# a1q123456/image_stitching

Measured on AMD Instinct MI355X. Metric: 4K frames stitched/sec, higher is better.
Workload: dtype u8

## Files before the change

image_stitching_amd/csrc/orb.hip:

```cpp
#include "common.h"
#include "dev_math.h"
#include <algorithm>
#include <chrono>
#include <cmath>

#define ORB_MAX_LEVELS 16
#define ORB_BORDER 32

namespace {

struct LevelDesc {
    int w, h;
    int pp;
    int sp;
    size_t pad_off;
    size_t map_off;
    float scale;
    int nfeat;
    int n2;
    int tiles_x, tiles_y, tile_off;
    int cap1, cand_off;
    int cap2, fin_off;
    int tab_off;
};
// ... 312 lines not shown
#pragma unroll
        for (int k = 0; k < FT_WR + 1; k++) {
            if ((ball[k] >> lane) & 1ull) {
                const int r = k < FT_WR ? r0 + k : r0 + (lane >> 1), c = k < FT_WR ? lane : FT_COLS + (lane & 1);
                queue[base + __popcll(ball[k] & below)] = (unsigned short)(r * (FT_COLS + 2) + c);
            }
            base += __popcll(ball[k]);
        }
    }
    __syncthreads();
    for (int q = t; q < qcount; q += 256) {
        const int i = queue[q], r = i / (FT_COLS + 2), c = i - r * (FT_COLS + 2);
        const int fsv = fast_score_full(g + (r + 3) * FG_PITCH + (c + FG_COL0), FG_PITCH, L.fast_t);
        sc[r * SP + c] = (uint8_t)fsv;
#ifdef MIS_ORB_STATS
        if (fsv) atomicAdd(&g_orb_stats[3], 1ull);
#endif
    }
    __syncthreads();
    lh[t] = 0;
    {
        const int nq = qcount;
        for (int q0 = 0; q0 < nq; q0 += 256) {
            const int q = q0 + t;
            bool keep = false;
            int x = 0, y = 0, v = 0;
            if (q < nq) {
                const int i = queue[q], r = i / (FT_COLS + 2), c = i - r * (FT_COLS + 2);
                const uint8_t* s_ = sc + r * SP + c;
                v = s_[0];
                x = x0 - 1 + c; y = y0 - 1 + r;
                keep = v && r >= 1 && r <= FT_ROWS && c >= 1 && c <= FT_COLS && x >= L.edge && x < d.w - L.edge && y >= L.edge && y < d.h - L.edge &&
                       v > s_[-1] && v > s_[1] && v > s_[-SP - 1] && v > s_[-SP] && v > s_[-SP + 1] && v > s_[SP - 1] && v > s_[SP] && v > s_[SP + 1];
            }
            const unsigned long long m = __ballot(keep);
            int base = 0;
            if ((t & 63) == 0 && m) base = atomicAdd(&lcount, __popcll(m));
            base = __shfl(base, 0);
            if (keep) {
                const int j = base + __popcll(m & ((1ull << (t & 63)) - 1ull));
                lxy[j] = (uint32_t)x | ((uint32_t)y << 16); lsc[j] = (uint8_t)v;
            }
        }
    }
    __syncthreads();
    const int n = lcount;
    const int tile = d.tile_off + blockIdx.y * d.tiles_x + blockIdx.x;
    if (t == 0) tile_cnt[tile] = n;
    if (n == 0) return;
    for (int j = t; j < n; j += 256) {
        atomicAdd(&lh[lsc[j]], 1);
        surv_xy[(size_t)tile * FT_SLOTS + j] = lxy[j]; surv_sc[(size_t)tile * FT_SLOTS + j] = lsc[j];
    }
    __syncthreads();
    if (lh[t]) atomicAdd(&hist[((lz * HIST_COPIES) + ((blockIdx.x + blockIdx.y) & (HIST_COPIES - 1))) * 256 + t], lh[t]);
}

__global__ __launch_bounds__(256) void fast_cut_kernel(Levels L, const int* hist, int* thr, int* flags, size_t ws) {
    __shared__ int suf[256];
    __shared__ int s_thr;
    const int l = blockIdx.x, t = threadIdx.x;
    WS_OFF(hist, blockIdx.y, ws); WS_OFF(thr, blockIdx.y, ws); WS_OFF(flags, blockIdx.y, ws);
    const LevelDesc& d = L.d[l];
    int hsum = 0;
    for (int c = 0; c < HIST_COPIES; c++) hsum += hist[(l * HIST_COPIES + c) * 256 + t];
    suf[t] = t ? hsum : 0;
    __syncthreads();
    for (int o = 1; o < 256; o <<= 1) {
        int add = t + o < 256 ? suf[t + o] : 0;
        __syncthreads();
        suf[t] += add;
        __syncthreads();
    }
    if (t == 0) s_thr = d.n2 == 0 ? 256 : 1;
    __syncthreads();
    if (d.n2 > 0 && suf[1] > d.n2 && t >= 1 && suf[t] >= d.n2 && (t == 255 || suf[t + 1] < d.n2)) s_thr = t;
    __syncthreads();
    if (t == 0) {
        thr[l] = s_thr;
        if (s_thr < 256 && suf[s_thr] > d.cap1) atomicOr(&flags[0], 1);
    }
}

constexpr int CT_TILES = 16;
__global__ __launch_bounds__(256) void compact_kernel(Levels L, const int* tile_cnt, const uint32_t* surv_xy, const uint8_t* surv_sc, const int* thr,
                                                      int* cnt1, uint32_t* cand_xy, float* cand_resp, size_t ws) {
    __shared__ int s_cnt[CT_TILES], s_off[CT_TILES];
    __shared__ int s_base;
    const int l = blockIdx.y, t = threadIdx.x, lane = t & 63, wave = t >> 6;
    WS_OFF(tile_cnt, blockIdx.z, ws); WS_OFF(surv_xy, blockIdx.z, ws); WS_OFF(surv_sc, blockIdx.z, ws); WS_OFF(thr, blockIdx.z, ws);
    WS_OFF(cnt1, blockIdx.z, ws); WS_OFF(cand_xy, blockIdx.z, ws); WS_OFF(cand_resp, blockIdx.z, ws);
    const LevelDesc& d = L.d[l];
    const int ntiles = d.tiles_x * d.tiles_y, first = blockIdx.x * CT_TILES;
    if (first >= ntiles) return;
    const int th = thr[l];
    for (int k = 0; k < CT_TILES / 4; k++) {
        const int slot = wave * (CT_TILES / 4) + k, til = first + slot;
        int cnt = 0;
        if (til < ntiles) {
            const int tile = d.tile_off + til, n = tile_cnt[tile];
            for (int j0 = 0; j0 < n; j0 += 64) {
                const int j = j0 + lane;
                const int v = j < n ? surv_sc[(size_t)tile * FT_SLOTS + j] : 0;
                cnt += __popcll(__ballot(v >= th && v > 0));
            }
        }
        if (lane == 0) s_cnt[slot] = cnt;
    }
    __syncthreads();
    if (t == 0) {
        int tot = 0;
        for (int k = 0; k < CT_TILES; k++) { s_off[k] = tot; tot += s_cnt[k]; }
        s_base = tot ? atomicAdd(&cnt1[l], tot) : 0;
    }
    __syncthreads();
    for (int k = 0; k < CT_TILES / 4; k++) {
        const int slot = wave * (CT_TILES / 4) + k, til = first + slot;
        if (til >= ntiles || s_cnt[slot] == 0) continue;
        const int tile = d.tile_off + til, n = tile_cnt[tile];
        int run = s_base + s_off[slot];
        for (int j0 = 0; j0 < n; j0 += 64) {
            const int j = j0 + lane;
            const int v = j < n ? surv_sc[(size_t)tile * FT_SLOTS + j] : 0;
            const bool keep = v >= th && v > 0;
            const unsigned long long m = __ballot(keep);
            if (keep) {
                const int i = run + __popcll(m & ((1ull << lane) - 1ull));
                if (i < d.cap1) { cand_xy[d.cand_off + i] = surv_xy[(size_t)tile * FT_SLOTS + j]; cand_resp[d.cand_off + i] = (float)v; }
            }
            run += __popcll(m);
        }
    }
}

__global__ void nms_raster_kernel(LevelDesc d, const int* tile_cnt, const uint32_t* surv_xy, const uint8_t* surv_sc, uint8_t* nms) {
    const int ntiles = d.tiles_x * d.tiles_y;
    for (int tl = blockIdx.x; tl < ntiles; tl += gridDim.x) {
        const int tile = d.tile_off + tl, n = tile_cnt[tile];
        for (int j = threadIdx.x; j < n; j += blockDim.x) {
            uint32_t xy = surv_xy[(size_t)tile * FT_SLOTS + j];
            nms[d.map_off + (size_t)(xy >> 16) * d.sp + (xy & 0xffff)] = surv_sc[(size_t)tile * FT_SLOTS + j];
        }
    }
}

__global__ __launch_bounds__(256) void harris_kernel(Levels L, const uint8_t* pad, const int* cnt1, const uint32_t* cand_xy, float* cand_resp, size_t ws) {
    const LevelDesc& d = L.d[blockIdx.y];
    WS_OFF(pad, blockIdx.z, ws); WS_OFF(cnt1, blockIdx.z, ws); WS_OFF(cand_xy, blockIdx.z, ws); WS_OFF(cand_resp, blockIdx.z, ws);
    int i = blockIdx.x * 256 + threadIdx.x;
    int n = min(cnt1[blockIdx.y], d.cap1);
    if (i >= n) return;
    uint32_t xy = cand_xy[d.cand_off + i];
    int x = xy & 0xffff, y = xy >> 16;
    const int pp = d.pp;
    const uint8_t* q0 = pad + d.pad_off + (size_t)(y + ORB_BORDER - 4) * pp + (x + ORB_BORDER - 4);
    const unsigned sh = (unsigned)((uintptr_t)q0 & 3u);
    const uint8_t* a0 = q0 - sh;
    int px[9][9];
#pragma unroll
    for (int r = 0; r < 9; r++) {
        const unsigned* row = reinterpret_cast<const unsigned*>(a0 + (size_t)r * pp);
        const unsigned d0 = row[0], d1 = row[1], d2 = row[2];
        const unsigned w0 = __builtin_amdgcn_alignbyte(d1, d0, sh), w1 = __builtin_amdgcn_alignbyte(d2, d1, sh), w2 = __builtin_amdgcn_alignbyte(0u, d2, sh);
#pragma unroll
        for (int k = 0; k < 4; k++) { px[r][k] = (int)((w0 >> (8 * k)) & 255u); px[r][4 + k] = (int)((w1 >> (8 * k)) & 255u); }
        px[r][8] = (int)(w2 & 255u);
    }
    int a = 0, b = 0, c = 0;
#pragma unroll
    for (int by = 0; by < 7; by++)
#pragma unroll
        for (int bx = 0; bx < 7; bx++) {
            const int Ix = (px[by + 1][bx + 2] - px[by + 1][bx]) * 2 + (px[by][bx + 2] - px[by][bx]) + (px[by + 2][bx + 2] - px[by + 2][bx]);
            const int Iy = (px[by + 2][bx + 1] - px[by][bx + 1]) * 2 + (px[by + 2][bx] - px[by][bx]) + (px[by + 2][bx + 2] - px[by][bx + 2]);
            a += Ix * Ix; b += Iy * Iy; c += Ix * Iy;
        }
    const float scale = 1.f / ((1 << 2) * 7 * 255.f);
    const float scale_sq_sq = scale * scale * scale * scale;
    float fa = (float)a, fb = (float)b, fc = (float)c;
    float s1 = fa * fb, s2 = fc * fc;
    float s3 = 0.04f * (fa + fb);
    s3 = s3 * (fa + fb);
    cand_resp[d.cand_off + i] = ((s1 - s2) - s3) * scale_sq_sq;
}

__device__ __forceinline__ uint32_t fkey(float f) {
    uint32_t u = __float_as_uint(f);
    return (u & 0x80000000u) ? ~u : (u | 0x80000000u);
}

__global__ __launch_bounds__(1024) void select_rank_kernel(Levels L, const int* cnt1, const uint32_t* cand_xy, const float* cand_resp,
                                                            int* cnt2, uint32_t* fin_xy, float* fin_resp, int* flags, int use_harris, size_t ws) {
    WS_OFF(cnt1, blockIdx.y, ws); WS_OFF(cand_xy, blockIdx.y, ws); WS_OFF(cand_resp, blockIdx.y, ws); WS_OFF(cnt2, blockIdx.y, ws);
    WS_OFF(fin_xy, blockIdx.y, ws); WS_OFF(fin_resp, blockIdx.y, ws); WS_OFF(flags, blockIdx.y, ws);
    __shared__ int hist[256];
    __shared__ uint32_t s_prefix, s_mask;
    __shared__ int s_k, s_m;
    __shared__ uint32_t kkey[4096], kxy[4096];
    const int l = blockIdx.x, t = threadIdx.x;
    const LevelDesc& d = L.d[l];
    const int n = min(cnt1[l], d.cap1);
    const uint32_t* xy = cand_xy + d.cand_off;
    const float* rs = cand_resp + d.cand_off;
    const int N = d.nfeat;
    if (N == 0) { if (t == 0) cnt2[l] = 0; return; }
    if (n <= 4096) {
        int P = 1;
        while (P < n) P <<= 1;
        for (int i = t; i < P; i += 1024) {
            if (i < n) { kkey[i] = fkey(rs[i]); kxy[i] = xy[i]; }
            else { kkey[i] = 0; kxy[i] = 0xffffffffu; }
        }
        __syncthreads();
        for (int k = 2; k <= P; k <<= 1)
            for (int j = k >> 1; j > 0; j >>= 1) {
                for (int i = t; i < P; i += 1024) {
                    const int ixj = i ^ j;
                    if (ixj > i) {
                        const uint32_t ka = kkey[i], kb = kkey[ixj], pa = kxy[i], pb = kxy[ixj];
                        const bool a_first = ka > kb || (ka == kb && pa < pb);
                        const bool descending_block = (i & k) == 0;
                        if (a_first != descending_block) { kkey[i] = kb; kkey[ixj] = ka; kxy[i] = pb; kxy[ixj] = pa; }
                    }
                }
                __syncthreads();
            }
        const uint32_t cutk = (use_harris && n > N) ? kkey[N - 1] : 0u;
        if (t == 0) s_m = 0;
        __syncthreads();
        for (int i = t; i < n; i += 1024)
            if (kkey[i] >= cutk && (i == n - 1 || kkey[i + 1] < cutk)) s_m = i + 1;
        __syncthreads();
        const int m = s_m;
        if (m > d.cap2) { if (t == 0) { atomicOr(&flags[0], 2); cnt2[l] = 0; } return; }
        for (int i = t; i < m; i += 1024) {
            fin_xy[d.fin_off + i] = kxy[i];
            const uint32_t ki = kkey[i], uu = (ki & 0x80000000u) ? (ki & 0x7fffffffu) : ~ki;
            fin_resp[d.fin_off + i] = __uint_as_float(uu);
        }
        if (t == 0) cnt2[l] = m;
        return;
    }
    uint32_t cut = 0;
    if (use_harris && n > N) {
        if (t == 0) { s_prefix = 0; s_mask = 0; s_k = N; }
        __syncthreads();
        for (int shift = 24; shift >= 0; shift -= 8) {
            if (t < 256) hist[t] = 0;
            __syncthreads();
            uint32_t prefix = s_prefix, mask = s_mask;
            for (int i = t; i < n; i += 1024) {
                uint32_t k = fkey(rs[i]);
                if ((k & mask) == prefix) atomicAdd(&hist[(k >> shift) & 255], 1);
            }
            __syncthreads();
            if (t == 0) {
                int k = s_k, b = 255;
                for (; b > 0; b--) { if (hist[b] >= k) break; k -= hist[b]; }
                s_k = k; s_prefix = prefix | ((uint32_t)b << shift); s_mask = mask | (0xffu << shift);
            }
            __syncthreads();
        }
        cut = s_prefix;
    }
    if (t == 0) s_m = 0;
    __syncthreads();
    for (int i = t; i < n; i += 1024) {
        uint32_t k = fkey(rs[i]);
        if (k >= cut) {
            int j = atomicAdd(&s_m, 1);
            if (j < 4096) { kkey[j] = k; kxy[j] = xy[i]; }
        }
    }
    __syncthreads();
    int m = s_m;
    if (m > d.cap2 || m > 4096) { if (t == 0) { atomicOr(&flags[0], 2); cnt2[l] = 0; } return; }
    for (int i = t; i < m; i += 1024) {
        uint32_t ki = kkey[i], pi = kxy[i];
        uint32_t yi = (pi >> 16), xi = pi & 0xffff;
        uint32_t oi = (yi << 16) | xi;
        int r = 0;
        for (int j = 0; j < m; j++) {
            uint32_t kj = kkey[j], pj = kxy[j];
            uint32_t oj = ((pj >> 16) << 16) | (pj & 0xffff);
            r += (kj > ki) || (kj == ki && oj < oi);
        }
        fin_xy[d.fin_off + r] = pi;
        uint32_t u = (ki & 0x80000000u) ? (ki & 0x7fffffffu) : ~ki;
        fin_resp[d.fin_off + r] = __uint_as_float(u);
    }
    if (t == 0) cnt2[l] = m;
}

__global__ __launch_bounds__(256) void assemble_kernel(Levels L, const int* cnt2, const uint32_t* fin_xy, const float* fin_resp, OrbIO io, int cap_out, size_t ws) {
    const int fr = blockIdx.y;
    WS_OFF(cnt2, fr, ws); WS_OFF(fin_xy, fr, ws); WS_OFF(fin_resp, fr, ws);
    MisKeyPoint* kps = io.kps[fr];
    int* n_out = io.n_dev[fr];
    const int j = blockIdx.x * 4 + (threadIdx.x >> 6), lane = threadIdx.x & 63;
    int base = 0, l = 0, total = 0;
    {
        int c[ORB_MAX_LEVELS];
#pragma unroll
        for (int k = 0; k < ORB_MAX_LEVELS; k++) c[k] = k < L.n ? cnt2[min(k, L.n - 1)] : 0;
#pragma unroll
        for (int k = 0; k < ORB_MAX_LEVELS; k++) {
            if (j >= total + c[k]) { base = total + c[k]; l = k + 1; }
            total += c[k];
        }
    }
    if (blockIdx.x == 0 && threadIdx.x == 0) *n_out = min(total, cap_out);
    if (j >= total || j >= cap_out) return;
    const LevelDesc& d = L.d[l];
    const int i = j - base;
    uint32_t xy = fin_xy[d.fin_off + i];
    int x = xy & 0xffff, y = xy >> 16;
    if (lane == 0) {
        MisKeyPoint kp;
        kp.x = (float)x * d.scale; kp.y = (float)y * d.scale;
        kp.size = (float)L.patch * d.scale;
        kp.angle = 0.f;
        kp.response = fin_resp[d.fin_off + i];
        kp.octave = l;
        kps[base + i] = kp;
    }
}

__global__ __launch_bounds__(256) void blur_kernel(Levels L, const uint8_t* pad, uint8_t* blur) {
    constexpr int TR = 32, TP = 80;
    __shared__ __attribute__((aligned(16))) uint8_t tile[(TR + 6) * TP];
    __shared__ __attribute__((aligned(16))) uint16_t hbuf[(TR + 6) * 64];
    const LevelDesc& d = L.d[blockIdx.z];
    const int pw = d.w + 2 * ORB_BORDER, ph = d.h + 2 * ORB_BORDER;
    const int tx0 = blockIdx.x * 64, ty0 = blockIdx.y * TR, t = threadIdx.x;
    if (tx0 >= pw || ty0 >= ph) return;
    const uint8_t* src = pad + d.pad_off;
    uint8_t* dst = blur + d.pad_off;
    for (int i = t; i < (TR + 6) * (TP / 4); i += 256) {
        const int r = i / (TP / 4), c = i - r * (TP / 4);
        const int sy = min(max(ty0 + r - 3, 0), ph - 1);
        int sx = tx0 - 4 + 4 * c;
        sx = min(max(sx, 0), d.pp - 4);
        reinterpret_cast<unsigned*>(tile)[i] = *reinterpret_cast<const unsigned*>(src + (size_t)sy * d.pp + sx);
    }
    __syncthreads();
    const int kq[7] = {18, 34, 48, 56, 48, 34, 18};
    for (int i = t; i < (TR + 6) * 16; i += 256) {
        const int r = i >> 4, cg = i & 15;
        const unsigned* p = reinterpret_cast<const unsigned*>(tile + r * TP + 4 * cg);
        const unsigned w0 = p[0], w1 = p[1], w2 = p[2];
        int b[12];
#pragma unroll
        for (int k = 0; k < 4; k++) { b[k] = (w0 >> (8 * k)) & 255; b[4 + k] = (w1 >> (8 * k)) & 255; b[8 + k] = (w2 >> (8 * k)) & 255; }
        unsigned short o[4];
#pragma unroll
        for (int k = 0; k < 4; k++) {
            int acc = 0;
#pragma unroll
            for (int j = 0; j < 7; j++) acc += kq[j] * b[k + 1 + j];
            o[k] = (unsigned short)acc;
        }
        *reinterpret_cast<uint2*>(hbuf + r * 64 + 4 * cg) = make_uint2(o[0] | ((unsigned)o[1] << 16), o[2] | ((unsigned)o[3] << 16));
    }
    __syncthreads();
    const int c = t & 63, px = tx0 + c;
    if (px >= pw) return;
    const int r0 = (t >> 6) * (TR / 4);
    int hv[TR / 4 + 6];
#pragma unroll
    for (int j = 0; j < TR / 4 + 6; j++) hv[j] = hbuf[(r0 + j) * 64 + c];
#pragma unroll
    for (int k = 0; k < TR / 4; k++) {
        const int r = r0 + k, py = ty0 + r;
        if (py >= ph) break;
        const int x = px - ORB_BORDER, y = py - ORB_BORDER;
        uint8_t o;
        if ((unsigned)x < (unsigned)d.w && (unsigned)y < (unsigned)d.h) {
            int acc = 0;
#pragma unroll
            for (int j = 0; j < 7; j++) acc += kq[j] * hv[k + j];
            o = (uint8_t)((acc + (1 << 15)) >> 16);
        } else o = tile[(r + 3) * TP + c + 4];
        dst[(size_t)py * d.pp + px] = o;
    }
}

constexpr int DD_R = 28, DD_P = DD_R + 3, DD_N = 2 * DD_P + 1, DD_ROW_DW = (DD_N + 3 + 3) / 4, DD_PITCH = 4 * DD_ROW_DW + 4;
constexpr int ORB_MAX_PATCH = 40;
static_assert(8 * (ORB_MAX_PATCH / 2) * (ORB_MAX_PATCH / 2) < (2 * DD_R + 1) * (2 * DD_R + 1), "round(sqrt(2) h) <= DD_R: every sample lies in the staged patch");
static_assert(3 + ORB_BORDER >= DD_P, "the staged patch lies inside the padded level");
struct UMax16 { int v[16]; };
__global__ __launch_bounds__(256) void describe_direct_kernel(Levels L, const uint8_t* pad, OrbIO io, const int8_t* pattern, const int* umax, UMax16 um16, size_t ws) {
    __shared__ __attribute__((aligned(16))) uint8_t patch[4][DD_N * DD_PITCH];
    const int wave = threadIdx.x >> 6, lane = threadIdx.x & 63;
    const int i = blockIdx.x * 4 + wave, fr = blockIdx.y;
    WS_OFF(pad, fr, ws);
    MisKeyPoint* kps = io.kps[fr];
    const int* n_ptr = io.n_dev[fr];
    uint8_t* desc = io.desc[fr];
    if (i >= *n_ptr) return;
    const MisKeyPoint kp = kps[i];
    const LevelDesc& d = L.d[kp.octave];
    const float inv = 1.f / d.scale;
    const int cx = mis_round_f(kp.x * inv), cy = mis_round_f(kp.y * inv);
    const int pp = d.pp;
    const uint8_t* org = pad + d.pad_off + (size_t)(cy + ORB_BORDER - DD_P) * pp + (cx + ORB_BORDER - DD_P);
    const int shift = (int)((uintptr_t)org & 3);
    const uint8_t* abase = org - shift;
    uint8_t* P = patch[wave];
    for (int k = lane; k < DD_N * DD_ROW_DW; k += 64) {
        const int r = k / DD_ROW_DW, c = k - r * DD_ROW_DW;
        reinterpret_cast<unsigned*>(P + r * DD_PITCH)[c] = *reinterpret_cast<const unsigned*>(abase + (size_t)r * pp + 4 * c);
    }
    __builtin_amdgcn_fence(__ATOMIC_ACQ_REL, "wavefront");
    __builtin_amdgcn_wave_barrier();
    const int c0 = DD_P * DD_PITCH + DD_P + shift;
    float kp_angle;
    {
        const int hp = L.half_patch;
        const uint8_t* ctr = P + c0;
        int m01 = 0, m10 = 0;
        const int u = lane - hp;
        if (lane <= 2 * hp) {
            m10 = u * ctr[u];
            if (hp <= 15) {
#pragma unroll 3
                for (int v = 1; v <= hp; ++v) {
                    const int vp = ctr[u + v * DD_PITCH], vm = ctr[u - v * DD_PITCH];
                    const bool in = abs(u) <= um16.v[v];
                    m10 += in ? u * (vp + vm) : 0;
                    m01 += in ? v * (vp - vm) : 0;
                }
            } else {
                for (int v = 1; v <= hp; ++v) {
                    if (abs(u) <= umax[v]) {
                        const int vp = ctr[u + v * DD_PITCH], vm = ctr[u - v * DD_PITCH];
                        m10 += u * (vp + vm);
                        m01 += v * (vp - vm);
                    }
                }
            }
        }
#pragma unroll
        for (int o = 32; o > 0; o >>= 1) { m01 += __shfl_xor(m01, o); m10 += __shfl_xor(m10, o); }
        kp_angle = mis_fast_atan2((float)m01, (float)m10);
        if (lane == 0) kps[i].angle = kp_angle;
    }
    float ang = kp_angle * (float)(3.14159265358979323846 / 180.f);
    float sa, ca;
    mis_sincosf(ang, &sa, &ca);
    const int b = lane & 31, h = lane >> 5;
    const int8_t* pat = pattern + b * 32 + h * 16;
    const unsigned* P32 = reinterpret_cast<const unsigned*>(P);
    auto blurred = [&](int ix, int iy) {
        const int a = c0 + (iy - 3) * DD_PITCH + (ix - 3);
        const bool inside = (unsigned)(cx + ix) < (unsigned)d.w && (unsigned)(cy + iy) < (unsigned)d.h;
        const unsigned* q = P32 + (a >> 2);
        const unsigned sh = (unsigned)(a & 3) << 3;
        const int kq[7] = {18, 34, 48, 56, 48, 34, 18};
        unsigned acc = 0, centre = 0;
#pragma unroll
        for (int j = 0; j < 7; j++) {
            const unsigned d0 = q[j * (DD_PITCH / 4)], d1 = q[j * (DD_PITCH / 4) + 1], d2 = q[j * (DD_PITCH / 4) + 2];
            const unsigned lo = __builtin_amdgcn_alignbit(d1, d0, sh), hi = __builtin_amdgcn_alignbit(d2, d1, sh);
            const unsigned hs = __builtin_amdgcn_udot4(lo, 0x38302212u, __builtin_amdgcn_udot4(hi, 0x00122230u, 0u, false), false);
            acc += (unsigned)kq[j] * hs;
            if (j == 3) centre = lo >> 24;
        }
        return inside ? (int)((acc + (1u << 15)) >> 16) : (int)centre;
    };
    int val = 0;
#pragma unroll 1
    for (int bit = 0; bit < 4; bit++) {
        float x0 = (float)pat[4 * bit], y0 = (float)pat[4 * bit + 1], x1 = (float)pat[4 * bit + 2], y1 = (float)pat[4 * bit + 3];
        int ix0 = mis_round_f(x0 * ca - y0 * sa), iy0 = mis_round_f(x0 * sa + y0 * ca);
        int ix1 = mis_round_f(x1 * ca - y1 * sa), iy1 = mis_round_f(x1 * sa + y1 * ca);
        const int t0 = blurred(ix0, iy0), t1 = blurred(ix1, iy1);
        val |= (t0 < t1) << (bit + 4 * h);
    }
    val |= __shfl_xor(val, 32);
    if (h == 0) desc[(size_t)i * 32 + b] = (uint8_t)val;
}

constexpr int ORB_GATHER_MAX = 96;
struct GatherPtrs { const int* p[ORB_GATHER_MAX]; };
__global__ void gather_ints_kernel(GatherPtrs g, int n, int* __restrict__ out) {
    const int i = blockIdx.x * blockDim.x + threadIdx.x;
    if (i < n) out[i] = *g.p[i];
}

}

struct MisOrb {
    MisContext* ctx = nullptr;
    void (*enqueued_cb)(void*) = nullptr;
    void* enqueued_user = nullptr;
    bool knn_armed = false;
    int knn_n = 0, knn_range_width = -1, knn_rank = 0, knn_world = 1;
    bool knn_has_mask = false;
    std::vector<uint8_t> knn_mask;
    OwnedEvent ev_counts;
    MisOrbParams p;
    int max_w = 0, max_h = 0;
    int cur_w = 0, cur_h = 0;
    Levels L;
    Work w;
    size_t ws_stride = 0;
    int ws_frames = 0;
    int umax_host[64] = {0};
    int8_t pattern_host[1024] = {0};
    void* mem = nullptr;
    size_t pad_bytes = 0, map_bytes = 0;
    int cand_total = 0, fin_total = 0, tab_total = 0, surv_total = 0, out_cap = 0;
    std::vector<int> tab_host;
    int* host_counts = nullptr;
};

namespace {

void linear_exact_coeffs(int dlen, int slen, int* ofs, int* m1) {
    double inv = (double)dlen / (double)slen, scale = 1.0 / inv;
    for (int i = 0; i < dlen; i++) {
        double v = ((double)i + 0.5) * scale - 0.5;
        int iv = (int)floor(v);
        if (iv < 0) { ofs[i] = 0; m1[i] = 0; }
        else if (iv >= slen - 1) { ofs[i] = slen - 1; m1[i] = 0; }
        else { ofs[i] = iv; m1[i] = (int)lrint((v - (double)iv) * 256.0); }
    }
}

constexpr int ORB_MAX_LEVEL_FEATURES = 2048 - 128;

inline float level_scale(const MisOrbParams& p, int l) { return (float)pow((double)p.scale_factor, (double)l); }
inline int level_dim(int len, float sc) { return (int)lrint((double)((float)len / sc)); }

void level_budgets(const MisOrbParams& p, int* nfeat) {
    float factor = (float)(1.0 / (double)p.scale_factor);
    float nd = (float)p.nfeatures * (1 - factor) / (1 - (float)pow((double)factor, (double)p.nlevels));
    int sum = 0;
    for (int l = 0; l < p.nlevels - 1; l++) { nfeat[l] = (int)lrintf(nd); sum += nfeat[l]; nd *= factor; }
    nfeat[p.nlevels - 1] = std::max(p.nfeatures - sum, 0);
}

int check_level_sizes(MisContext* ctx, const MisOrbParams& p, int w, int h) {
    for (int l = 0; l < p.nlevels; l++) {
        const float sc = level_scale(p, l);
        MIS_CHECK(ctx, level_dim(w, sc) >= 1 && level_dim(h, sc) >= 1, MIS_E_UNSUPPORTED,
                  "ORB level %d of a %dx%d frame is empty (scale_factor %g, nlevels %d)", l, w, h, (double)p.scale_factor, p.nlevels);
    }
    return MIS_OK;
}

void plan_levels(MisOrb* o, int w, int h) {
    Levels& L = o->L;
    const MisOrbParams& p = o->p;
    L.n = p.nlevels; L.fast_t = p.fast_threshold; L.patch = p.patch_size; L.half_patch = p.patch_size / 2; L.edge = p.edge_threshold;
    size_t pad_off = 0, map_off = 0;
    int cand_off = 0, fin_off = 0, tab_off = 0, surv_off = 0;
    int nfeat[ORB_MAX_LEVELS];
    level_budgets(p, nfeat);
    for (int l = 0; l < L.n; l++) {
        LevelDesc& d = L.d[l];
        float sc = level_scale(p, l);
        d.scale = sc;
        d.w = level_dim(w, sc);
        d.h = level_dim(h, sc);
        d.pp = (int)mis_align_up((size_t)d.w + 2 * ORB_BORDER, 64);
        d.sp = (int)mis_align_up((size_t)d.w, 64);
        d.pad_off = pad_off; pad_off += (size_t)d.pp * (d.h + 2 * ORB_BORDER);
        d.map_off = map_off; map_off += (size_t)d.sp * d.h;
        d.nfeat = nfeat[l];
        d.n2 = p.score_type == 0 ? 2 * d.nfeat : d.nfeat;
        d.tiles_x = (d.w + FT_COLS - 1) / FT_COLS; d.tiles_y = (d.h + FT_ROWS - 1) / FT_ROWS;
        d.tile_off = surv_off; surv_off += d.tiles_x * d.tiles_y;
        d.cap1 = 4 * d.n2 + 4096;
        d.cap2 = std::min(d.nfeat + 128, 2048);
        d.cand_off = cand_off; cand_off += d.cap1;
        d.fin_off = fin_off; fin_off += d.cap2;
        d.tab_off = tab_off; tab_off += (2 * ((d.w + 3) & ~3) + 2 * d.h + 3) & ~3;
    }
    o->pad_bytes = pad_off; o->map_bytes = map_off; o->cand_total = cand_off; o->fin_total = fin_off; o->tab_total = tab_off; o->surv_total = surv_off;
    o->tab_host.assign(tab_off, 0);
    for (int l = 1; l < L.n; l++) {
        int* t = o->tab_host.data() + L.d[l].tab_off;
        const int dw4 = (L.d[l].w + 3) & ~3;
        linear_exact_coeffs(L.d[l].w, L.d[l - 1].w, t, t + dw4);
        linear_exact_coeffs(L.d[l].h, L.d[l - 1].h, t + 2 * dw4, t + 2 * dw4 + L.d[l].h);
    }
}

int upload_tables(MisOrb* o) {
    MisContext* ctx = o->ctx;
    if (o->tab_total)
        MIS_HIP(ctx, hipMemcpyAsync(o->w.tab, o->tab_host.data(), sizeof(int) * o->tab_total, hipMemcpyHostToDevice, ctx->stream));
    MIS_HIP(ctx, hipStreamSynchronize(ctx->stream));
    return MIS_OK;
}

int enqueue_detect_group(MisOrb* o, const DevView* img, int w, int h, MisFeatures* out, int ng) {
    MisContext* ctx = o->ctx;
    const Levels& L = o->L;
    const Work& W = o->w;
    hipStream_t st = ctx->stream;
    const LevelDesc& d0 = L.d[0];
    const size_t ws = o->ws_stride;
    const unsigned nf = (unsigned)ng;
    OrbIO io;
    for (int k = 0; k < ORB_BATCH; k++) {
        const int q = k < ng ? k : 0;
        io.src[k] = (const uint8_t*)img[q].data; io.sstride[k] = img[q].stride;
        io.aligned[k] = (img[q].stride % 4 == 0) && ((uintptr_t)img[q].data % 4 == 0);
        io.kps[k] = out[q].keypoints; io.n_dev[k] = mis_feat_count(&out[q], o->out_cap);
        io.desc[k] = (uint8_t*)out[q].descriptors;
    }
    MIS_HIP(ctx, hipMemset2DAsync(W.hist, ws ? ws : sizeof(int) * (256 * HIST_COPIES * ORB_MAX_LEVELS + 4 * ORB_MAX_LEVELS), 0,
                                  sizeof(int) * (256 * HIST_COPIES * ORB_MAX_LEVELS + 4 * ORB_MAX_LEVELS), nf, st));
    hipLaunchKernelGGL(gray_kernel, dim3((w + 1023) / 1024, (h + GRAY_ROWS - 1) / GRAY_ROWS, nf), dim3(256), 0, st, io, w, h, W.pad + d0.pad_off, d0.pp, ws);
    for (int l = 1; l < L.n; l++) {
        const LevelDesc &s = L.d[l - 1], &d = L.d[l];
        hipLaunchKernelGGL(resize_kernel, dim3((d.w + 255) / 256, (d.h + 4 * RS_ROWS - 1) / (4 * RS_ROWS), nf), dim3(256), 0, st, W.pad + s.pad_off, s.w, s.h, s.pp, W.pad + d.pad_off, d.w,
                           d.h, d.pp, W.tab + d.tab_off, ws);
    }
    const int pw0 = d0.w + 2 * ORB_BORDER;
    hipLaunchKernelGGL((border_kernel<true>), dim3((d0.h * 16 + 255) / 256, 1, L.n * nf), dim3(256), 0, st, L, W.pad, ws);
    hipLaunchKernelGGL((border_kernel<false>), dim3((pw0 + 1023) / 1024, 2 * ORB_BORDER / 4, L.n * nf), dim3(256), 0, st, L, W.pad, ws);
    dim3 gmap((d0.w + FT_COLS - 1) / FT_COLS, (d0.h + FT_ROWS - 1) / FT_ROWS, L.n * nf);
    hipLaunchKernelGGL(fast_nms_kernel, gmap, dim3(256), 0, st, L, W.pad, W.hist, W.tile_cnt, W.surv_xy, W.surv_sc, ws);
    hipLaunchKernelGGL(fast_cut_kernel, dim3(L.n, nf), dim3(256), 0, st, L, W.hist, W.thr, W.flags, ws);
    hipLaunchKernelGGL(compact_kernel, dim3((d0.tiles_x * d0.tiles_y + CT_TILES - 1) / CT_TILES, L.n, nf), dim3(256), 0, st, L, W.tile_cnt, W.surv_xy, W.surv_sc, W.thr, W.cnt1,
                       W.cand_xy, W.cand_resp, ws);
    const int use_harris = o->p.score_type == 0;
    if (use_harris)
        hipLaunchKernelGGL(harris_kernel, dim3((L.d[0].cap1 + 255) / 256, L.n, nf), dim3(256), 0, st, L, W.pad, W.cnt1, W.cand_xy, W.cand_resp, ws);
    hipLaunchKernelGGL(select_rank_kernel, dim3(L.n, nf), dim3(1024), 0, st, L, W.cnt1, W.cand_xy, W.cand_resp, W.cnt2, W.fin_xy, W.fin_resp, W.flags,
                       use_harris, ws);
    hipLaunchKernelGGL(assemble_kernel, dim3((o->out_cap + 3) / 4, nf), dim3(256), 0, st, L, W.cnt2, W.fin_xy, W.fin_resp, io, o->out_cap, ws);
    UMax16 um16;
    for (int v = 0; v < 16; v++) um16.v[v] = o->umax_host[v];
    hipLaunchKernelGGL(describe_direct_kernel, dim3((o->out_cap + 3) / 4, nf), dim3(256), 0, st, L, W.pad, io, W.pattern, W.umax, um16, ws);
    MIS_HIP(ctx, hipGetLastError());
    return MIS_OK;
}

int check_image(MisOrb* o, const MisImage* bgr) {
    MisContext* ctx = o->ctx;
    MIS_CHECK(ctx, bgr && bgr->data, MIS_E_INVALID, "null image");
    MIS_CHECK(ctx, bgr->dtype == MIS_U8 && bgr->channels == 3, MIS_E_UNSUPPORTED, "ORB input must be 8UC3 (BGR)");
    MIS_CHECK(ctx, bgr->width <= o->max_w && bgr->height <= o->max_h && bgr->width >= 64 && bgr->height >= 64, MIS_E_INVALID,
              "image %dx%d outside the finder's range (64x64 .. %dx%d)", bgr->width, bgr->height, o->max_w, o->max_h);
    return MIS_OK;
}

int replan_if_needed(MisOrb* o, int w, int h) {
    if (w == o->cur_w && h == o->cur_h) return MIS_OK;
    const int rc = check_level_sizes(o->ctx, o->p, w, h);
    if (rc != MIS_OK) return rc;
    MIS_HIP(o->ctx, hipStreamSynchronize(o->ctx->stream));
    plan_levels(o, w, h);
    o->cur_w = w; o->cur_h = h;
    return upload_tables(o);
}

int orb_alloc_workspace(MisOrb* o, int frames) {
    MisContext* ctx = o->ctx;
    size_t off = 0;
    auto carve = [&](size_t bytes) { size_t o_ = off; off += mis_align_up(bytes, 256); return o_; };
    size_t o_pad = carve(o->pad_bytes);
    size_t o_hist = carve(sizeof(int) * (256 * HIST_COPIES * ORB_MAX_LEVELS + 4 * ORB_MAX_LEVELS)), o_flags = carve(256);
    size_t o_sxy = carve(sizeof(uint32_t) * FT_SLOTS * (size_t)o->surv_total), o_ssc = carve(FT_SLOTS * (size_t)o->surv_total), o_tc = carve(sizeof(int) * (size_t)o->surv_total);
    size_t o_cxy = carve(sizeof(uint32_t) * o->cand_total), o_cr = carve(sizeof(float) * o->cand_total);
    size_t o_fxy = carve(sizeof(uint32_t) * o->fin_total), o_fr = carve(sizeof(float) * o->fin_total);
    size_t o_tab = carve(sizeof(int) * (o->tab_total + 4)), o_umax = carve(sizeof(int) * 64), o_pat = carve(1024);
    const size_t tail = mis_align_up(o->map_bytes, 256) + mis_align_up(o->pad_bytes, 256);
    void* mem = nullptr;
    if (hipMalloc(&mem, off * (size_t)frames + tail) != hipSuccess) return mis_set_error(ctx, MIS_E_NOMEM, "hipMalloc of %zu bytes failed", off * (size_t)frames + tail);
    o->mem = mem; o->ws_stride = off; o->ws_frames = frames;
    uint8_t* m = (uint8_t*)o->mem;
    uint8_t* shared = m + off * (size_t)frames;
    Work& W = o->w;
    W.pad = m + o_pad; W.nms = shared; W.blur = shared + mis_align_up(o->map_bytes, 256);
    W.hist = (int*)(m + o_hist); W.thr = W.hist + 256 * HIST_COPIES * ORB_MAX_LEVELS; W.cnt1 = W.thr + ORB_MAX_LEVELS; W.cnt2 = W.cnt1 + ORB_MAX_LEVELS;
    W.surv_xy = (uint32_t*)(m + o_sxy); W.surv_sc = m + o_ssc; W.tile_cnt = (int*)(m + o_tc);
    W.flags = (int*)(m + o_flags);
    W.cand_xy = (uint32_t*)(m + o_cxy); W.cand_resp = (float*)(m + o_cr); W.fin_xy = (uint32_t*)(m + o_fxy); W.fin_resp = (float*)(m + o_fr);
    W.tab = (int*)(m + o_tab); W.umax = (int*)(m + o_umax); W.pattern = (int8_t*)(m + o_pat);
    return MIS_OK;
}

int orb_init_workspace(MisOrb* o) {
    MisContext* ctx = o->ctx;
    const Work& W = o->w;
    MIS_HIP(ctx, hipMemcpyAsync(W.umax, o->umax_host, sizeof(o->umax_host), hipMemcpyHostToDevice, ctx->stream));
    MIS_HIP(ctx, hipMemcpyAsync(W.pattern, o->pattern_host, sizeof(o->pattern_host), hipMemcpyHostToDevice, ctx->stream));
    MIS_HIP(ctx, hipMemset2DAsync(W.flags, o->ws_stride, 0, 256, (size_t)o->ws_frames, ctx->stream));
    MIS_HIP(ctx, hipStreamSynchronize(ctx->stream));
    return upload_tables(o);
}

int orb_ensure_frames(MisOrb* o, int frames) {
    frames = std::min(frames, ORB_BATCH);
    if (o->ws_frames >= frames) return MIS_OK;
    MisContext* ctx = o->ctx;
    MIS_HIP(ctx, hipStreamSynchronize(ctx->stream));
    void* old = o->mem;
    const Work oldw = o->w;
    const size_t olds = o->ws_stride;
    const int oldf = o->ws_frames;
    int rc = MIS_E_NOMEM;
    for (int f = frames; f > oldf; f = std::max(oldf, f / 2)) {
        if ((rc = orb_alloc_workspace(o, f)) == MIS_OK) break;
    }
    if (rc != MIS_OK) {
        o->mem = old; o->w = oldw; o->ws_stride = olds; o->ws_frames = oldf;
        return oldf >= 1 ? MIS_OK : rc;
    }
    if (old) MIS_HIP(ctx, hipFree(old));
    return orb_init_workspace(o);
}

int gather_counts_and_flags(MisOrb* o, MisFeatures* out, int n, int* flags) {
    MisContext* ctx = o->ctx;
    const int total = n + o->ws_frames;
// ... 233 lines not shown
```

Baseline: 3504.

## Fuse Harris into rank select, assemble into describe, flatten compact grid

Harris scoring moves into select_rank_kernel and now uses packed 16-bit sdot2 arithmetic. Keypoint assembly is folded into describe_direct_kernel, and compact_kernel runs over a flat tile range spanning all levels. The bitonic sort does its inner steps in registers with wave shuffles, so it needs fewer shared-memory passes and barriers. Together these drop two kernel launches and several global round-trips. The cost is that Harris work is serialized into one 1024-thread block per level, and the kernels are more complex.

```diff
diff --git a/image_stitching_amd/csrc/orb.hip b/image_stitching_amd/csrc/orb.hip
--- a/image_stitching_amd/csrc/orb.hip
+++ b/image_stitching_amd/csrc/orb.hip
@@ -418,51 +418,77 @@
     }
 }
 
-constexpr int CT_TILES = 16;
-__global__ __launch_bounds__(256) void compact_kernel(Levels L, const int* tile_cnt, const uint32_t* surv_xy, const uint8_t* surv_sc, const int* thr,
+constexpr int CT_TILES = 16, CT_WT = CT_TILES / 4;
+__global__ __launch_bounds__(256) void compact_kernel(Levels L, int ntiles, const int* tile_cnt, const uint32_t* surv_xy, const uint8_t* surv_sc, const int* thr,
                                                       int* cnt1, uint32_t* cand_xy, float* cand_resp, size_t ws) {
-    __shared__ int s_cnt[CT_TILES], s_off[CT_TILES];
-    __shared__ int s_base;
-    const int l = blockIdx.y, t = threadIdx.x, lane = t & 63, wave = t >> 6;
-    WS_OFF(tile_cnt, blockIdx.z, ws); WS_OFF(surv_xy, blockIdx.z, ws); WS_OFF(surv_sc, blockIdx.z, ws); WS_OFF(thr, blockIdx.z, ws);
-    WS_OFF(cnt1, blockIdx.z, ws); WS_OFF(cand_xy, blockIdx.z, ws); WS_OFF(cand_resp, blockIdx.z, ws);
-    const LevelDesc& d = L.d[l];
-    const int ntiles = d.tiles_x * d.tiles_y, first = blockIdx.x * CT_TILES;
-    if (first >= ntiles) return;
-    const int th = thr[l];
-    for (int k = 0; k < CT_TILES / 4; k++) {
-        const int slot = wave * (CT_TILES / 4) + k, til = first + slot;
-        int cnt = 0;
-        if (til < ntiles) {
-            const int tile = d.tile_off + til, n = tile_cnt[tile];
-            for (int j0 = 0; j0 < n; j0 += 64) {
-                const int j = j0 + lane;
-                const int v = j < n ? surv_sc[(size_t)tile * FT_SLOTS + j] : 0;
-                cnt += __popcll(__ballot(v >= th && v > 0));
-            }
-        }
-        if (lane == 0) s_cnt[slot] = cnt;
+    __shared__ int s_cnt[CT_TILES], s_off[CT_TILES], s_lvl[CT_TILES];
+    const int t = threadIdx.x, lane = t & 63, wave = __builtin_amdgcn_readfirstlane(t >> 6);
+    WS_OFF(tile_cnt, blockIdx.y, ws); WS_OFF(surv_xy, blockIdx.y, ws); WS_OFF(surv_sc, blockIdx.y, ws); WS_OFF(thr, blockIdx.y, ws);
+    WS_OFF(cnt1, blockIdx.y, ws); WS_OFF(cand_xy, blockIdx.y, ws); WS_OFF(cand_resp, blockIdx.y, ws);
+    const int first = blockIdx.x * CT_TILES + wave * CT_WT;
+    int lv[CT_WT], n[CT_WT], th[CT_WT], v0[CT_WT], cnt[CT_WT];
+    uint32_t p0[CT_WT];
+#pragma unroll
+    for (int k = 0; k < CT_WT; k++) {
+        const int tile = first + k;
+        lv[k] = -1; n[k] = 0; th[k] = 256;
+        if (tile < ntiles) {
+            int l = 0;
+            for (int q = 1; q < L.n; q++) l += tile >= L.d[q].tile_off;
+            lv[k] = l; n[k] = tile_cnt[tile]; th[k] = thr[l];
+        }
+    }
+#pragma unroll
+    for (int k = 0; k < CT_WT; k++) {
+        const size_t at = (size_t)(first + k) * FT_SLOTS + lane;
+        v0[k] = lane < n[k] ? surv_sc[at] : 0;
+        p0[k] = lane < n[k] ? surv_xy[at] : 0u;
+    }
+#pragma unroll
+    for (int k = 0; k < CT_WT; k++) {
+        cnt[k] = __popcll(__ballot(v0[k] >= th[k] && v0[k] > 0));
+        for (int j0 = 64; j0 < n[k]; j0 += 64) {
+            const int j = j0 + lane;
+            const int v = j < n[k] ? surv_sc[(size_t)(first + k) * FT_SLOTS + j] : 0;
+            cnt[k] += __popcll(__ballot(v >= th[k] && v > 0));
+        }
+        if (lane == 0) { s_cnt[wave * CT_WT + k] = cnt[k]; s_lvl[wave * CT_WT + k] = lv[k]; }
     }
     __syncthreads();
     if (t == 0) {
-        int tot = 0;
-        for (int k = 0; k < CT_TILES; k++) { s_off[k] = tot; tot += s_cnt[k]; }
-        s_base = tot ? atomicAdd(&cnt1[l], tot) : 0;
-    }
-    __syncthreads();
-    for (int k = 0; k < CT_TILES / 4; k++) {
-        const int slot = wave * (CT_TILES / 4) + k, til = first + slot;
-        if (til >= ntiles || s_cnt[slot] == 0) continue;
-        const int tile = d.tile_off + til, n = tile_cnt[tile];
-        int run = s_base + s_off[slot];
-        for (int j0 = 0; j0 < n; j0 += 64) {
-            const int j = j0 + lane;
-            const int v = j < n ? surv_sc[(size_t)tile * FT_SLOTS + j] : 0;
-            const bool keep = v >= th && v > 0;
+        for (int k = 0; k < CT_TILES;) {
+            const int l = s_lvl[k];
+            int k1 = k, tot = 0;
+            for (; k1 < CT_TILES && s_lvl[k1] == l; k1++) { s_off[k1] = tot; tot += s_cnt[k1]; }
+            const int base = tot ? atomicAdd(&cnt1[l], tot) : 0;
+            for (int q = k; q < k1; q++) s_off[q] += base;
+            k = k1;
+        }
+    }
+    __syncthreads();
+#pragma unroll
+    for (int k = 0; k < CT_WT; k++) {
+        if (cnt[k] == 0) continue;
+        const LevelDesc& d = L.d[lv[k]];
+        int run = s_off[wave * CT_WT + k];
+        {
+            const bool keep = v0[k] >= th[k] && v0[k] > 0;
             const unsigned long long m = __ballot(keep);
             if (keep) {
                 const int i = run + __popcll(m & ((1ull << lane) - 1ull));
-                if (i < d.cap1) { cand_xy[d.cand_off + i] = surv_xy[(size_t)tile * FT_SLOTS + j]; cand_resp[d.cand_off + i] = (float)v; }
+                if (i < d.cap1) { cand_xy[d.cand_off + i] = p0[k]; cand_resp[d.cand_off + i] = (float)v0[k]; }
+            }
+            run += __popcll(m);
+        }
+        for (int j0 = 64; j0 < n[k]; j0 += 64) {
+            const int j = j0 + lane;
+            const size_t at = (size_t)(first + k) * FT_SLOTS + j;
+            const int v = j < n[k] ? surv_sc[at] : 0;
+            const bool keep = v >= th[k] && v > 0;
+            const unsigned long long m = __ballot(keep);
+            if (keep) {
+                const int i = run + __popcll(m & ((1ull << lane) - 1ull));
+                if (i < d.cap1) { cand_xy[d.cand_off + i] = surv_xy[at]; cand_resp[d.cand_off + i] = (float)v; }
             }
             run += __popcll(m);
         }
@@ -480,44 +506,48 @@
     }
 }
 
-__global__ __launch_bounds__(256) void harris_kernel(Levels L, const uint8_t* pad, const int* cnt1, const uint32_t* cand_xy, float* cand_resp, size_t ws) {
-    const LevelDesc& d = L.d[blockIdx.y];
-    WS_OFF(pad, blockIdx.z, ws); WS_OFF(cnt1, blockIdx.z, ws); WS_OFF(cand_xy, blockIdx.z, ws); WS_OFF(cand_resp, blockIdx.z, ws);
-    int i = blockIdx.x * 256 + threadIdx.x;
-    int n = min(cnt1[blockIdx.y], d.cap1);
-    if (i >= n) return;
-    uint32_t xy = cand_xy[d.cand_off + i];
-    int x = xy & 0xffff, y = xy >> 16;
-    const int pp = d.pp;
-    const uint8_t* q0 = pad + d.pad_off + (size_t)(y + ORB_BORDER - 4) * pp + (x + ORB_BORDER - 4);
+struct __attribute__((aligned(4))) HarrisRow { unsigned d[3]; };
+__device__ __forceinline__ float harris_response(const uint8_t* lvl, int pp, int x, int y) {
+    const uint8_t* q0 = lvl + (size_t)(y + ORB_BORDER - 4) * pp + (x + ORB_BORDER - 4);
     const unsigned sh = (unsigned)((uintptr_t)q0 & 3u);
     const uint8_t* a0 = q0 - sh;
-    int px[9][9];
+    unsigned w[9][3];
 #pragma unroll
     for (int r = 0; r < 9; r++) {
-        const unsigned* row = reinterpret_cast<const unsigned*>(a0 + (size_t)r * pp);
-        const unsigned d0 = row[0], d1 = row[1], d2 = row[2];
-        const unsigned w0 = __builtin_amdgcn_alignbyte(d1, d0, sh), w1 = __builtin_amdgcn_alignbyte(d2, d1, sh), w2 = __builtin_amdgcn_alignbyte(0u, d2, sh);
-#pragma unroll
-        for (int k = 0; k < 4; k++) { px[r][k] = (int)((w0 >> (8 * k)) & 255u); px[r][4 + k] = (int)((w1 >> (8 * k)) & 255u); }
-        px[r][8] = (int)(w2 & 255u);
-    }
+        const HarrisRow row = *reinterpret_cast<const HarrisRow*>(a0 + (size_t)r * pp);
+        const unsigned d0 = row.d[0], d1 = row.d[1], d2 = row.d[2];
+        w[r][0] = __builtin_amdgcn_alignbyte(d1, d0, sh); w[r][1] = __builtin_amdgcn_alignbyte(d2, d1, sh); w[r][2] = __builtin_amdgcn_alignbyte(0u, d2, sh);
+    }
+    typedef short s16x2 __attribute__((ext_vector_type(2)));
+    s16x2 dx[3][4], sm[3][4];
+    auto prepare = [&](int r) {
+        auto pair = [](unsigned hi, unsigned lo, unsigned sel) { return __builtin_bit_cast(s16x2, __builtin_amdgcn_perm(hi, lo, sel)); };
+        const unsigned w0 = w[r][0], w1 = w[r][1], w2 = w[r][2] & 255u;
+        const s16x2 e[5] = {pair(0u, w0, 0x0c010c00u), pair(0u, w0, 0x0c030c02u), pair(0u, w1, 0x0c010c00u), pair(0u, w1, 0x0c030c02u), __builtin_bit_cast(s16x2, w2)};
+        const s16x2 o[4] = {pair(0u, w0, 0x0c020c01u), pair(w1, w0, 0x0c040c03u), pair(0u, w1, 0x0c020c01u), pair(w2, w1, 0x0c040c03u)};
+#pragma unroll
+        for (int k = 0; k < 4; k++) { dx[r % 3][k] = e[k + 1] - e[k]; sm[r % 3][k] = e[k] + e[k + 1] + o[k] + o[k]; }
+    };
+    prepare(0); prepare(1);
     int a = 0, b = 0, c = 0;
 #pragma unroll
-    for (int by = 0; by < 7; by++)
-#pragma unroll
-        for (int bx = 0; bx < 7; bx++) {
-            const int Ix = (px[by + 1][bx + 2] - px[by + 1][bx]) * 2 + (px[by][bx + 2] - px[by][bx]) + (px[by + 2][bx + 2] - px[by + 2][bx]);
-            const int Iy = (px[by + 2][bx + 1] - px[by][bx + 1]) * 2 + (px[by + 2][bx] - px[by][bx]) + (px[by + 2][bx + 2] - px[by][bx + 2]);
-            a += Ix * Ix; b += Iy * Iy; c += Ix * Iy;
-        }
+    for (int by = 0; by < 7; by++) {
+        prepare(by + 2);
+        const int r0 = by % 3, r1 = (by + 1) % 3, r2 = (by + 2) % 3;
+#pragma unroll
+        for (int k = 0; k < 4; k++) {
+            s16x2 Ix = dx[r0][k] + dx[r2][k] + dx[r1][k] + dx[r1][k], Iy = sm[r2][k] - sm[r0][k];
+            if (k == 3) { Ix.y = 0; Iy.y = 0; }
+            a = __builtin_amdgcn_sdot2(Ix, Ix, a, false); b = __builtin_amdgcn_sdot2(Iy, Iy, b, false); c = __builtin_amdgcn_sdot2(Ix, Iy, c, false);
+        }
+    }
     const float scale = 1.f / ((1 << 2) * 7 * 255.f);
     const float scale_sq_sq = scale * scale * scale * scale;
     float fa = (float)a, fb = (float)b, fc = (float)c;
     float s1 = fa * fb, s2 = fc * fc;
     float s3 = 0.04f * (fa + fb);
     s3 = s3 * (fa + fb);
-    cand_resp[d.cand_off + i] = ((s1 - s2) - s3) * scale_sq_sq;
+    return ((s1 - s2) - s3) * scale_sq_sq;
 }
 
 __device__ __forceinline__ uint32_t fkey(float f) {
@@ -525,8 +555,9 @@
     return (u & 0x80000000u) ? ~u : (u | 0x80000000u);
 }
 
-__global__ __launch_bounds__(1024) void select_rank_kernel(Levels L, const int* cnt1, const uint32_t* cand_xy, const float* cand_resp,
+__global__ __launch_bounds__(1024) void select_rank_kernel(Levels L, const uint8_t* pad, const int* cnt1, const uint32_t* cand_xy, float* cand_resp,
                                                             int* cnt2, uint32_t* fin_xy, float* fin_resp, int* flags, int use_harris, size_t ws) {
+    WS_OFF(pad, blockIdx.y, ws);
     WS_OFF(cnt1, blockIdx.y, ws); WS_OFF(cand_xy, blockIdx.y, ws); WS_OFF(cand_resp, blockIdx.y, ws); WS_OFF(cnt2, blockIdx.y, ws);
     WS_OFF(fin_xy, blockIdx.y, ws); WS_OFF(fin_resp, blockIdx.y, ws); WS_OFF(flags, blockIdx.y, ws);
     __shared__ int hist[256];
@@ -537,30 +568,80 @@
     const LevelDesc& d = L.d[l];
     const int n = min(cnt1[l], d.cap1);
     const uint32_t* xy = cand_xy + d.cand_off;
-    const float* rs = cand_resp + d.cand_off;
+    float* rs = cand_resp + d.cand_off;
+    const uint8_t* lvl = pad + d.pad_off;
     const int N = d.nfeat;
     if (N == 0) { if (t == 0) cnt2[l] = 0; return; }
+    if (use_harris) {
+        uint32_t pnext = t < n ? xy[t] : 0u;
+#pragma unroll 1
+        for (int i = t; i < n; i += 1024) {
+            const uint32_t p = pnext;
+            if (i + 1024 < n) pnext = xy[i + 1024];
+            const float r = harris_response(lvl, d.pp, (int)(p & 0xffffu), (int)(p >> 16));
+            if (n <= 4096) { kkey[i] = fkey(r); kxy[i] = p; }
+            else rs[i] = r;
+        }
+    }
     if (n <= 4096) {
-        int P = 1;
+        int P = 64;
         while (P < n) P <<= 1;
         for (int i = t; i < P; i += 1024) {
-            if (i < n) { kkey[i] = fkey(rs[i]); kxy[i] = xy[i]; }
-            else { kkey[i] = 0; kxy[i] = 0xffffffffu; }
-        }
-        __syncthreads();
-        for (int k = 2; k <= P; k <<= 1)
-            for (int j = k >> 1; j > 0; j >>= 1) {
-                for (int i = t; i < P; i += 1024) {
-                    const int ixj = i ^ j;
-                    if (ixj > i) {
-                        const uint32_t ka = kkey[i], kb = kkey[ixj], pa = kxy[i], pb = kxy[ixj];
-                        const bool a_first = ka > kb || (ka == kb && pa < pb);
-                        const bool descending_block = (i & k) == 0;
-                        if (a_first != descending_block) { kkey[i] = kb; kkey[ixj] = ka; kxy[i] = pb; kxy[ixj] = pa; }
-                    }
+            if (i >= n) { kkey[i] = 0; kxy[i] = 0xffffffffu; }
+            else if (!use_harris) { kkey[i] = fkey(rs[i]); kxy[i] = xy[i]; }
+        }
+        const int nm = max(P >> 10, 1);
+        uint32_t ek[4], ep[4];
+#pragma unroll
+        for (int m = 0; m < 4; m++) {
+            const int i = t + 1024 * m;
+            ek[m] = 0; ep[m] = 0xffffffffu;
+            if (i < P) { ek[m] = kkey[i]; ep[m] = kxy[i]; }
+        }
+        auto lane_steps = [&](int k, int j0) {
+            for (int j = j0; j > 0; j >>= 1) {
+#pragma unroll
+                for (int m = 0; m < 4; m++) {
+                    if (m >= nm) break;
+                    const int i = t + 1024 * m;
+                    const uint32_t ok = __shfl_xor(ek[m], j), op = __shfl_xor(ep[m], j);
+                    const bool mine_first = ek[m] > ok || (ek[m] == ok && ep[m] < op);
+                    const bool want_first = ((i & j) == 0) == ((i & k) == 0);
+                    if (mine_first != want_first) { ek[m] = ok; ep[m] = op; }
+                }
+            }
+        };
+        for (int k = 2; k <= 64; k <<= 1) lane_steps(k, k >> 1);
+        for (int k = 128; k <= P; k <<= 1) {
+#pragma unroll
+            for (int m = 0; m < 4; m++) {
+                const int i = t + 1024 * m;
+                if (i < P) { kkey[i] = ek[m]; kxy[i] = ep[m]; }
+            }
+            __syncthreads();
+            for (int j = k >> 1; j >= 64; j >>= 1) {
+                for (int q = t; q < (P >> 1); q += 1024) {
+                    const int i = ((q & ~(j - 1)) << 1) | (q & (j - 1)), ixj = i | j;
+                    const uint32_t ka = kkey[i], kb = kkey[ixj], pa = kxy[i], pb = kxy[ixj];
+                    const bool a_first = ka > kb || (ka == kb && pa < pb);
+                    const bool descending_block = (i & k) == 0;
+                    if (a_first != descending_block) { kkey[i] = kb; kkey[ixj] = ka; kxy[i] = pb; kxy[ixj] = pa; }
                 }
                 __syncthreads();
             }
+#pragma unroll
+            for (int m = 0; m < 4; m++) {
+                const int i = t + 1024 * m;
+                if (i < P) { ek[m] = kkey[i]; ep[m] = kxy[i]; }
+            }
+            lane_steps(k, 32);
+        }
+#pragma unroll
+        for (int m = 0; m < 4; m++) {
+            const int i = t + 1024 * m;
+            if (i < P) { kkey[i] = ek[m]; kxy[i] = ep[m]; }
+        }
+        __syncthreads();
         const uint32_t cutk = (use_harris && n > N) ? kkey[N - 1] : 0u;
         if (t == 0) s_m = 0;
         __syncthreads();
@@ -577,6 +658,7 @@
         if (t == 0) cnt2[l] = m;
         return;
     }
+    __syncthreads();
     uint32_t cut = 0;
     if (use_harris && n > N) {
         if (t == 0) { s_prefix = 0; s_mask = 0; s_k = N; }
@@ -626,40 +708,6 @@
         fin_resp[d.fin_off + r] = __uint_as_float(u);
     }
     if (t == 0) cnt2[l] = m;
-}
-
-__global__ __launch_bounds__(256) void assemble_kernel(Levels L, const int* cnt2, const uint32_t* fin_xy, const float* fin_resp, OrbIO io, int cap_out, size_t ws) {
-    const int fr = blockIdx.y;
-    WS_OFF(cnt2, fr, ws); WS_OFF(fin_xy, fr, ws); WS_OFF(fin_resp, fr, ws);
-    MisKeyPoint* kps = io.kps[fr];
-    int* n_out = io.n_dev[fr];
-    const int j = blockIdx.x * 4 + (threadIdx.x >> 6), lane = threadIdx.x & 63;
-    int base = 0, l = 0, total = 0;
-    {
-        int c[ORB_MAX_LEVELS];
-#pragma unroll
-        for (int k = 0; k < ORB_MAX_LEVELS; k++) c[k] = k < L.n ? cnt2[min(k, L.n - 1)] : 0;
-#pragma unroll
-        for (int k = 0; k < ORB_MAX_LEVELS; k++) {
-            if (j >= total + c[k]) { base = total + c[k]; l = k + 1; }
-            total += c[k];
-        }
-    }
-    if (blockIdx.x == 0 && threadIdx.x == 0) *n_out = min(total, cap_out);
-    if (j >= total || j >= cap_out) return;
-    const LevelDesc& d = L.d[l];
-    const int i = j - base;
-    uint32_t xy = fin_xy[d.fin_off + i];
-    int x = xy & 0xffff, y = xy >> 16;
-    if (lane == 0) {
-        MisKeyPoint kp;
-        kp.x = (float)x * d.scale; kp.y = (float)y * d.scale;
-        kp.size = (float)L.patch * d.scale;
-        kp.angle = 0.f;
-        kp.response = fin_resp[d.fin_off + i];
-        kp.octave = l;
-        kps[base + i] = kp;
-    }
 }
 
 __global__ __launch_bounds__(256) void blur_kernel(Levels L, const uint8_t* pad, uint8_t* blur) {
@@ -726,19 +774,30 @@
 static_assert(8 * (ORB_MAX_PATCH / 2) * (ORB_MAX_PATCH / 2) < (2 * DD_R + 1) * (2 * DD_R + 1), "round(sqrt(2) h) <= DD_R: every sample lies in the staged patch");
 static_assert(3 + ORB_BORDER >= DD_P, "the staged patch lies inside the padded level");
 struct UMax16 { int v[16]; };
-__global__ __launch_bounds__(256) void describe_direct_kernel(Levels L, const uint8_t* pad, OrbIO io, const int8_t* pattern, const int* umax, UMax16 um16, size_t ws) {
+__global__ __launch_bounds__(256) void describe_direct_kernel(Levels L, const uint8_t* pad, const int* cnt2, const uint32_t* fin_xy, const float* fin_resp, OrbIO io, int cap_out,
+                                                              const int8_t* pattern, const int* umax, UMax16 um16, size_t ws) {
     __shared__ __attribute__((aligned(16))) uint8_t patch[4][DD_N * DD_PITCH];
-    const int wave = threadIdx.x >> 6, lane = threadIdx.x & 63;
+    const int wave = __builtin_amdgcn_readfirstlane(threadIdx.x >> 6), lane = threadIdx.x & 63;
     const int i = blockIdx.x * 4 + wave, fr = blockIdx.y;
-    WS_OFF(pad, fr, ws);
+    WS_OFF(pad, fr, ws); WS_OFF(cnt2, fr, ws); WS_OFF(fin_xy, fr, ws); WS_OFF(fin_resp, fr, ws);
     MisKeyPoint* kps = io.kps[fr];
-    const int* n_ptr = io.n_dev[fr];
     uint8_t* desc = io.desc[fr];
-    if (i >= *n_ptr) return;
-    const MisKeyPoint kp = kps[i];
-    const LevelDesc& d = L.d[kp.octave];
-    const float inv = 1.f / d.scale;
-    const int cx = mis_round_f(kp.x * inv), cy = mis_round_f(kp.y * inv);
+    int base = 0, l = 0, total = 0;
+#pragma unroll
+    for (int k = 0; k < ORB_MAX_LEVELS; k++) {
+        const int c = cnt2[k];
+        if (i >= total + c) { base = total + c; l = k + 1; }
+        total += c;
+    }
+    const int n_out = min(total, cap_out);
+    if (blockIdx.x == 0 && threadIdx.x == 0) *io.n_dev[fr] = n_out;
+    if (i >= n_out) return;
+    const LevelDesc& d = L.d[l];
+    const uint32_t kxy = fin_xy[d.fin_off + (i - base)];
+    float kresp = fin_resp[d.fin_off + (i - base)], kscale = d.scale;
+    int ksize = L.patch, lw = d.w, lh = d.h;
+    asm volatile("" : "+s"(kresp), "+s"(kscale), "+s"(ksize), "+s"(lw), "+s"(lh));
+    const int cx = (int)(kxy & 0xffffu), cy = (int)(kxy >> 16);
     const int pp = d.pp;
     const uint8_t* org = pad + d.pad_off + (size_t)(cy + ORB_BORDER - DD_P) * pp + (cx + ORB_BORDER - DD_P);
     const int shift = (int)((uintptr_t)org & 3);
@@ -780,7 +839,6 @@
 #pragma unroll
         for (int o = 32; o > 0; o >>= 1) { m01 += __shfl_xor(m01, o); m10 += __shfl_xor(m10, o); }
         kp_angle = mis_fast_atan2((float)m01, (float)m10);
-        if (lane == 0) kps[i].angle = kp_angle;
     }
     float ang = kp_angle * (float)(3.14159265358979323846 / 180.f);
     float sa, ca;
@@ -790,7 +848,7 @@
     const unsigned* P32 = reinterpret_cast<const unsigned*>(P);
     auto blurred = [&](int ix, int iy) {
         const int a = c0 + (iy - 3) * DD_PITCH + (ix - 3);
-        const bool inside = (unsigned)(cx + ix) < (unsigned)d.w && (unsigned)(cy + iy) < (unsigned)d.h;
+        const bool inside = (unsigned)(cx + ix) < (unsigned)lw && (unsigned)(cy + iy) < (unsigned)lh;
         const unsigned* q = P32 + (a >> 2);
         const unsigned sh = (unsigned)(a & 3) << 3;
         const int kq[7] = {18, 34, 48, 56, 48, 34, 18};
@@ -816,6 +874,15 @@
     }
     val |= __shfl_xor(val, 32);
     if (h == 0) desc[(size_t)i * 32 + b] = (uint8_t)val;
+    if (lane == 0) {
+        MisKeyPoint kp;
+        kp.x = (float)cx * kscale; kp.y = (float)cy * kscale;
+        kp.size = (float)ksize * kscale;
+        kp.angle = kp_angle;
+        kp.response = kresp;
+        kp.octave = l;
+        kps[i] = kp;
+    }
 }
 
 constexpr int ORB_GATHER_MAX = 96;
@@ -963,17 +1030,15 @@
     dim3 gmap((d0.w + FT_COLS - 1) / FT_COLS, (d0.h + FT_ROWS - 1) / FT_ROWS, L.n * nf);
     hipLaunchKernelGGL(fast_nms_kernel, gmap, dim3(256), 0, st, L, W.pad, W.hist, W.tile_cnt, W.surv_xy, W.surv_sc, ws);
     hipLaunchKernelGGL(fast_cut_kernel, dim3(L.n, nf), dim3(256), 0, st, L, W.hist, W.thr, W.flags, ws);
-    hipLaunchKernelGGL(compact_kernel, dim3((d0.tiles_x * d0.tiles_y + CT_TILES - 1) / CT_TILES, L.n, nf), dim3(256), 0, st, L, W.tile_cnt, W.surv_xy, W.surv_sc, W.thr, W.cnt1,
+    hipLaunchKernelGGL(compact_kernel, dim3((o->surv_total + CT_TILES - 1) / CT_TILES, nf), dim3(256), 0, st, L, o->surv_total, W.tile_cnt, W.surv_xy, W.surv_sc, W.thr, W.cnt1,
                        W.cand_xy, W.cand_resp, ws);
     const int use_harris = o->p.score_type == 0;
-    if (use_harris)
-        hipLaunchKernelGGL(harris_kernel, dim3((L.d[0].cap1 + 255) / 256, L.n, nf), dim3(256), 0, st, L, W.pad, W.cnt1, W.cand_xy, W.cand_resp, ws);
-    hipLaunchKernelGGL(select_rank_kernel, dim3(L.n, nf), dim3(1024), 0, st, L, W.cnt1, W.cand_xy, W.cand_resp, W.cnt2, W.fin_xy, W.fin_resp, W.flags,
+    hipLaunchKernelGGL(select_rank_kernel, dim3(L.n, nf), dim3(1024), 0, st, L, W.pad, W.cnt1, W.cand_xy, W.cand_resp, W.cnt2, W.fin_xy, W.fin_resp, W.flags,
                        use_harris, ws);
-    hipLaunchKernelGGL(assemble_kernel, dim3((o->out_cap + 3) / 4, nf), dim3(256), 0, st, L, W.cnt2, W.fin_xy, W.fin_resp, io, o->out_cap, ws);
     UMax16 um16;
     for (int v = 0; v < 16; v++) um16.v[v] = o->umax_host[v];
-    hipLaunchKernelGGL(describe_direct_kernel, dim3((o->out_cap + 3) / 4, nf), dim3(256), 0, st, L, W.pad, io, W.pattern, W.umax, um16, ws);
+    hipLaunchKernelGGL(describe_direct_kernel, dim3((o->out_cap + 3) / 4, nf), dim3(256), 0, st, L, W.pad, W.cnt2, W.fin_xy, W.fin_resp, io, o->out_cap, W.pattern, W.umax,
+                       um16, ws);
     MIS_HIP(ctx, hipGetLastError());
     return MIS_OK;
 }
```

New measurement: 3515 (median of 4 runs). No clear change (+0.3%).
